# lesliegaga/GPT-SoVITS

Measured on AMD Instinct MI355X. Metric: synthesised audio sec/sec (1/RTF), v2 pipeline, higher is better.
Workload: dtype f16

## Files before the change

### gpt-sovits_amd/csrc/conv_launch.h

```cpp
#pragma once
#include <stdlib.h>

#include <algorithm>
#include <type_traits>

#include "common.h"

namespace gsv {

int launch_gemm_sk(int dtype, const ConvArgs& a, hipStream_t s);
int launch_conv_wide(int dtype, const ConvArgs& a, hipStream_t s);
int launch_gemm_lds(int dtype, const ConvArgs& a, hipStream_t s);
int launch_conv_narrow(int dtype, const ConvArgs& a, hipStream_t s);
int launch_conv_lds(int dtype, const ConvArgs& a, hipStream_t s);

inline const char* env_switch(const char* name) { return getenv(name); }
inline long long env_number(const char* name, long long unset) { const char* v = env_switch(name); return v ? atoll(v) : unset; }
inline char env_first(const char* name) { const char* v = env_switch(name); return v ? v[0] : '\0'; }
struct ConvSwitches {
  bool no_conv_lds = env_switch("GSV_NO_CONV_LDS");
  bool trace_conv_gemm = env_switch("GSV_TRACE_CONV_GEMM");
  long long gemm_small_tiles = env_number("GSV_CONV_GEMM_SMALL_TILES", 64);
  bool no_gemm_sk = env_switch("GSV_NO_GEMM_SK");
  int sk_max_tiles = (int)env_number("GSV_SK_MAX_TILES", 160);
  bool gemm_t64 = env_first("GSV_GEMM_T64") != '0';
  int t64_slab = (int)env_number("GSV_T64_SLAB", 128);
  bool no_conv_wide = env_switch("GSV_NO_CONV_WIDE");
  int wide_waves = (int)env_number("GSV_WIDE_WAVES", 8);
  bool wide_prof = env_switch("GSV_WIDE_PROF");
  int gemm_xcd = env_first("GSV_GEMM_XCD") == '0' ? 0 : env_first("GSV_GEMM_XCD") == '1' ? 1 : 2;
  int gemm_waves = (int)env_number("GSV_GEMM_WAVES", 8);
  long long gemm_w8_max_tiles = env_number("GSV_GEMM_W8_MAX_TILES", 256);
  bool no_persist = env_switch("GSV_CONV_NO_PERSIST");
  bool no_persist64 = env_switch("GSV_CONV_NO_PERSIST64");
  int narrow_per_cu = std::max(1, (int)env_number("GSV_NARROW_PER_CU", 3));
  bool narrow_prof = env_switch("GSV_NARROW_PROF");
  bool no_half_tile = env_switch("GSV_CONV_NO_HALF_TILE");
  bool half_always = env_switch("GSV_CONV_HALF_ALWAYS");
  int half_waves = (int)env_number("GSV_CONV_HALF_WAVES", 8);
  int tile_waves = (int)env_number("GSV_CONV_TILE_WAVES", 8);
  bool no_conv_pair = env_switch("GSV_NO_CONV_PAIR");
  bool no_conv_pair64 = env_switch("GSV_NO_CONV_PAIR64");
  int pair_per_cu = std::max(1, (int)env_number("GSV_PAIR_PER_CU", 3));
};
inline const ConvSwitches& conv_switches() {
  static const ConvSwitches sw{};
  return sw;
}

template <auto Kern, int LdsCap, typename... Args>
int launch_routed(unsigned long long route, dim3 grid, dim3 block, size_t lds, hipStream_t s, Args... args) {
  if constexpr (LdsCap > 0) {
    static bool cap_set = false;
    if (!cap_set) {
      GSV_HIP(hipFuncSetAttribute((const void*)Kern, hipFuncAttributeMaxDynamicSharedMemorySize, LdsCap));
      cap_set = true;
    }
  }
  set_conv_route(route);
  GSV_LAUNCH(Kern, grid, block, lds, s, args...);
  return GSV_OK;
}
constexpr int LDS_CAP = 160 * 1024;

template <typename F> int with_flags(F&& f) { return f(); }
template <typename F, typename... Bools> int with_flags(F&& f, bool b, Bools... rest) {
  return with_flags([&](auto... tail) { return b ? f(std::true_type{}, tail...) : f(std::false_type{}, tail...); }, rest...);
}

template <int G> bool operands_aligned(const ConvArgs& a) {
  return a.ldx % G == 0 && a.ldw % G == 0 && (uintptr_t)a.x % 16 == 0 && (uintptr_t)a.w % 16 == 0;
}

struct TileStamps {
  unsigned long long* dev = nullptr;
  int calls = 0;
  unsigned long long* buffer(bool on) {
    if (on && !dev) { (void)hipMalloc((void**)&dev, 64 * 8); (void)hipMemset(dev, 0, 64 * 8); }
    return dev;
  }
  void report(hipStream_t s, int max_stamps, const char* fmt, ...) {
    if (!dev || ++calls != 3) return;
    (void)hipStreamSynchronize(s);
    unsigned long long hp[64];
    (void)hipMemcpy(hp, dev, sizeof(hp), hipMemcpyDeviceToHost);
    va_list ap;
    va_start(ap, fmt);
    vfprintf(stderr, fmt, ap);
    va_end(ap);
    for (int i = 1; i < max_stamps && hp[i]; ++i) fprintf(stderr, " %.2f", (double)(hp[i] - hp[0]) / 100.0);
    fprintf(stderr, "\n");
  }
};

}
```

### gpt-sovits_amd/csrc/conv_wide.hip

```cpp
#include "conv_launch.h"

namespace gsv {

namespace {

typedef _Float16 T;
typedef h8 F;
typedef _Float16 T4 __attribute__((ext_vector_type(4)));

__device__ __forceinline__ void mma32w(f16v& acc, const h8& a, const h8& b) { acc = __builtin_amdgcn_mfma_f32_32x32x16_f16(a, b, acc, 0, 0, 0); }
__device__ __forceinline__ h8 lrelu8w(h8 v, float s) { h8 t = v * (_Float16)s; return __builtin_elementwise_max(v, t); }
__device__ __forceinline__ h8 relu8w(h8 v) { return __builtin_elementwise_max(v, (h8){0, 0, 0, 0, 0, 0, 0, 0}); }

template <bool RES, bool ACCU, int NW>
__global__ __launch_bounds__(NW * 64) void conv_wide_f16_kernel(ConvArgs a, int rows_win, int ntiles) {
  constexpr int G = 8, KC = 16, CC = 128, CT = 128, TM = 2, TN = NW == 8 ? 2 : 4, WN = NW == 8 ? 4 : 2, NT = NW * 64;
  constexpr int LDX = CC + G, VPR = CC / G;
  constexpr int WLOADS = CT * VPR / NT;
  constexpr int XB = (306 * VPR + NT - 1) / NT;
  constexpr int LDO = CT + 4, PR = TN * 32, IPR = CT / 4, NI = PR * IPR / NT;
  extern __shared__ __attribute__((aligned(16))) unsigned char smem[];
  T* xs = (T*)smem;
  T* ws = xs + (size_t)306 * LDX;
  float* os = (float*)smem;
  static_assert((size_t)PR * LDO * 4 <= (size_t)306 * LDX * 2, "epilogue tile must fit in the window");
  const int tid = threadIdx.x, lane = tid & 63, wave = tid >> 6;
  const int r = lane & 31, h = lane >> 5;
  const int wm = wave / WN, wn = wave % WN;
  const T* __restrict__ x = (const T*)a.x;
  const T* __restrict__ w = (const T*)a.w;
  const int total = rows_win * VPR;
  const int ecg = tid % IPR, ec = 4 * ecg;
  f4 ebias = (f4){0.f, 0.f, 0.f, 0.f};
  if (a.bias) for (int j = 0; j < 4; ++j) ebias[j] = a.bias[ec + j];

  auto load_w = [&](int tap, F* regs) {
#pragma unroll
    for (int i = 0; i < WLOADS; ++i) {
      const int v = tid + i * NT;
      const int row = v / VPR, col = v - row * VPR;
      regs[i] = *(const F*)(w + (long long)row * a.ldw + (long long)tap * CC + col * G);
    }
  };
  auto store_w = [&](int buf, const F* regs) {
#pragma unroll
    for (int i = 0; i < WLOADS; ++i) {
      const int v = tid + i * NT;
      const int row = v / VPR, col = v - row * VPR;
      *(F*)(ws + ((size_t)buf * CT + row) * LDX + col * G) = regs[i];
    }
  };
  auto load_window = [&](int tile, F* regs) {
    const int win_start = tile * 256 - a.pad;
#pragma unroll
    for (int i = 0; i < XB; ++i) {
      const int v = min(tid + i * NT, total - 1);
      const int row = v / VPR, col = v - row * VPR;
      const int ti = win_start + row;
      const F val = *(const F*)(x + (long long)min(max(ti, 0), a.T_in - 1) * a.ldx + col * G);
      regs[i] = (ti >= 0 && ti < a.T_in) ? val : (F){0, 0, 0, 0, 0, 0, 0, 0};
    }
  };
  auto store_window = [&](const F* regs) {
#pragma unroll
    for (int i = 0; i < XB; ++i) {
      const int v = tid + i * NT;
      if (v < total) {
        const int row = v / VPR, col = v - row * VPR;
        F val = regs[i];
        if (a.pre_act == ACT_LRELU) val = lrelu8w(val, a.pre_slope);
        else if (a.pre_act == ACT_RELU) val = relu8w(val);
        *(F*)(xs + (size_t)row * LDX + col * G) = val;
      }
    }
  };
  int tile = blockIdx.x;
  {
    F first[XB], w0[WLOADS];
    load_window(min(tile, ntiles - 1), first);
    load_w(0, w0);
    store_window(first);
    store_w(0, w0);
  }
  lds_barrier();
  for (; tile < ntiles; tile += gridDim.x) {
    const int t0 = tile * 256;
    const bool pf = a.prof && blockIdx.x == 100 && tile == 100 + 3 * (int)gridDim.x && tid == 0;
    int pi = 0;
#define WSTAMP() do { if (pf) a.prof[pi++] = __builtin_amdgcn_s_memrealtime(); } while (0)
    WSTAMP();
    F nxt[XB];
    load_window(min(tile + (int)gridDim.x, ntiles - 1), nxt);
    T4 rv[RES ? NI : 1];
    auto load_res_pass = [&](int pass) {
#pragma unroll
      for (int e = 0; e < (RES ? NI : 0); ++e) {
        const int t = min(t0 + pass * PR + (tid + e * NT) / IPR, a.T_out - 1);
        rv[e] = *(const T4*)((const T*)a.res + (long long)t * a.ldr + ec);
      }
    };
    if (RES) load_res_pass(0);
    f16v acc[TM][TN];
#pragma unroll
    for (int m = 0; m < TM; ++m)
#pragma unroll
      for (int n = 0; n < TN; ++n)
#pragma unroll
        for (int i = 0; i < 16; ++i) acc[m][n][i] = 0.f;
    for (int tap = 0; tap < a.taps; ++tap) {
      const int buf = tap & 1;
      F wnx[WLOADS];
      const bool more = tap + 1 < a.taps;
      if (more) load_w(tap + 1, wnx);
      const int shift = tap * a.dil;
      const T* wb = ws + (size_t)buf * CT * LDX;
#pragma unroll 2
      for (int ks = 0; ks < CC / KC; ++ks) {
        const int kk = ks * KC + G * h;
        F af[TM], bf[TN];
#pragma unroll
        for (int m = 0; m < TM; ++m) af[m] = *(const F*)(wb + (size_t)((wm * TM + m) * 32 + r) * LDX + kk);
#pragma unroll
        for (int n = 0; n < TN; ++n) bf[n] = *(const F*)(xs + (size_t)((wn * TN + n) * 32 + r + shift) * LDX + kk);
#pragma unroll
        for (int m = 0; m < TM; ++m)
#pragma unroll
          for (int n = 0; n < TN; ++n) mma32w(acc[m][n], af[m], bf[n]);
      }
      if (more) {
        store_w(buf ^ 1, wnx);
        lds_barrier();
      }
      WSTAMP();
    }
#pragma unroll
    for (int pass = 0; pass < WN; ++pass) {
      lds_barrier();
      WSTAMP();
      if (wn == pass) {
#pragma unroll
        for (int m = 0; m < TM; ++m)
#pragma unroll
          for (int n = 0; n < TN; ++n) {
            const int tl = n * 32 + r;
#pragma unroll
            for (int g = 0; g < 4; ++g) {
              const int cl = (wm * TM + m) * 32 + 8 * g + 4 * h;
              *(f4*)(os + (size_t)tl * LDO + cl) = (f4){acc[m][n][4 * g], acc[m][n][4 * g + 1], acc[m][n][4 * g + 2], acc[m][n][4 * g + 3]};
            }
          }
      }
      WSTAMP();
      lds_barrier();
      WSTAMP();
      T4 ya[ACCU ? NI : 1];
#pragma unroll
      for (int e = 0; e < (ACCU ? NI : 0); ++e) {
        const int t = min(t0 + pass * PR + (tid + e * NT) / IPR, a.T_out - 1);
        ya[e] = *(const T4*)((const T*)a.y + (long long)t * a.ldy + ec);
      }
      auto items = [&](auto act_tag) {
#pragma unroll
        for (int e = 0; e < NI; ++e) {
          const int tl = (tid + e * NT) / IPR;
          const int t = t0 + pass * PR + tl;
          if (t >= a.T_out) continue;
          const f4 av = *(const f4*)(os + (size_t)tl * LDO + 4 * ecg);
          float v[4];
#pragma unroll
          for (int j = 0; j < 4; ++j) {
            float u = av[j] + ebias[j];
            if (RES) u += (float)rv[e][j];
            u *= a.scale;
            u = post_act_c<decltype(act_tag)::value>(a.post_act, u);
            if (ACCU) u += (float)ya[e][j];
            v[j] = u;
          }
          *(T4*)((T*)a.y + (long long)t * a.ldy + ec) = (T4){(T)v[0], (T)v[1], (T)v[2], (T)v[3]};
        }
      };
      GSV_ACT_DISPATCH(a.post_act, items);
      if (RES && pass + 1 < WN) load_res_pass(pass + 1);
      WSTAMP();
    }
    F w0[WLOADS];
    load_w(0, w0);
    lds_barrier();
    store_window(nxt);
    store_w(0, w0);
    lds_barrier();
    WSTAMP();
  }
}

}

int launch_conv_wide(int dtype, const ConvArgs& a, hipStream_t s) {
  const ConvSwitches& sw = conv_switches();
  if (sw.no_conv_wide || dtype != GSV_F16) return 1;
  if (a.Cin != 128 || a.Cout != 128 || a.Z != 1 || a.stride != 1 || a.ups_u > 0 || a.dil < 1 || a.gate || a.taps < 2) return 1;
  if (a.out_f32 || a.res_f32 || a.y_col0 != 0 || a.T_virt < 16384 || a.T_out != a.T_virt || a.T_in < 1) return 1;
  if (!operands_aligned<8>(a) || a.ldy % 4 != 0 || (a.res && a.ldr % 4 != 0)) return 1;
  const int span = (a.taps - 1) * a.dil;
  if (span > 50 || a.pad < 0 || a.pad > span) return 1;
  const int rows_win = 256 + span;
  const int ntiles = cdiv(a.T_virt, 256);
  const size_t lds = ((size_t)306 + 2 * 128) * 136 * 2;
  const int grid = std::min(ntiles, 256);
  static TileStamps stamps;
  ConvArgs b = a;
  b.prof = stamps.buffer(sw.wide_prof);
  GSV_RC(with_flags([&](auto R, auto A, auto W8) {
    constexpr int NW = W8.value ? 8 : 4;
    return launch_routed<conv_wide_f16_kernel<R.value, A.value, NW>, LDS_CAP>(
        route_code(ROUTE_CONV_WIDE, GSV_F16, NW, 0, 0, 0, 0, route_flags(R.value, A.value)), dim3(grid), dim3(NW * 64), lds, s, b, rows_win, ntiles);
  }, a.res != nullptr, a.accumulate != 0, sw.wide_waves == 8));
  stamps.report(s, 24, "[wide prof] taps %d:", a.taps);
  return GSV_OK;
}

}
```

Before: 2930.

## Give each wave a private epilogue scratch in the wide conv kernel

The block-wide epilogue made 4 passes, each with two block barriers. It is replaced by a per-wave epilogue in which every wave writes its accumulators to its own LDS scratch slice and drains it with only an lgkmcnt wait. Residual and accumulate reads are issued up front for all of a wave's rows. The weight reload for the next tile is folded into the last tap iteration and stored during the epilogue. The 4-wave variant is removed. A non-fused multiply-add is kept for specific elements to preserve exact rounding against a reference, which is an odd numerics-matching hack that adds fragility.

```diff
diff --git a/gpt-sovits_amd/csrc/conv_launch.h b/gpt-sovits_amd/csrc/conv_launch.h
--- a/gpt-sovits_amd/csrc/conv_launch.h
+++ b/gpt-sovits_amd/csrc/conv_launch.h
@@ -26,7 +26,6 @@
   bool gemm_t64 = env_first("GSV_GEMM_T64") != '0';
   int t64_slab = (int)env_number("GSV_T64_SLAB", 128);
   bool no_conv_wide = env_switch("GSV_NO_CONV_WIDE");
-  int wide_waves = (int)env_number("GSV_WIDE_WAVES", 8);
   bool wide_prof = env_switch("GSV_WIDE_PROF");
   int gemm_xcd = env_first("GSV_GEMM_XCD") == '0' ? 0 : env_first("GSV_GEMM_XCD") == '1' ? 1 : 2;
   int gemm_waves = (int)env_number("GSV_GEMM_WAVES", 8);
diff --git a/gpt-sovits_amd/csrc/conv_wide.hip b/gpt-sovits_amd/csrc/conv_wide.hip
--- a/gpt-sovits_amd/csrc/conv_wide.hip
+++ b/gpt-sovits_amd/csrc/conv_wide.hip
@@ -11,33 +11,41 @@
 __device__ __forceinline__ void mma32w(f16v& acc, const h8& a, const h8& b) { acc = __builtin_amdgcn_mfma_f32_32x32x16_f16(a, b, acc, 0, 0, 0); }
 __device__ __forceinline__ h8 lrelu8w(h8 v, float s) { h8 t = v * (_Float16)s; return __builtin_elementwise_max(v, t); }
 __device__ __forceinline__ h8 relu8w(h8 v) { return __builtin_elementwise_max(v, (h8){0, 0, 0, 0, 0, 0, 0, 0}); }
-
-template <bool RES, bool ACCU, int NW>
-__global__ __launch_bounds__(NW * 64) void conv_wide_f16_kernel(ConvArgs a, int rows_win, int ntiles) {
-  constexpr int G = 8, KC = 16, CC = 128, CT = 128, TM = 2, TN = NW == 8 ? 2 : 4, WN = NW == 8 ? 4 : 2, NT = NW * 64;
+__device__ __forceinline__ float mul_then_add(float u, float s, float y) {
+#pragma clang fp contract(off)
+  const float p = u * s;
+  return p + y;
+}
+__device__ __forceinline__ void wave_lds_wait() { asm volatile("s_waitcnt lgkmcnt(0)" ::: "memory"); }
+
+constexpr int WIDE_WAVES = 8;
+template <bool RES, bool ACCU>
+__global__ __launch_bounds__(WIDE_WAVES * 64) void conv_wide_f16_kernel(ConvArgs a, int rows_win, int ntiles) {
+  constexpr int G = 8, KC = 16, CC = 128, CT = 128, TM = 2, TN = 2, WN = 4, NW = WIDE_WAVES, NT = NW * 64;
   constexpr int LDX = CC + G, VPR = CC / G;
   constexpr int WLOADS = CT * VPR / NT;
   constexpr int XB = (306 * VPR + NT - 1) / NT;
-  constexpr int LDO = CT + 4, PR = TN * 32, IPR = CT / 4, NI = PR * IPR / NT;
+  constexpr int WC = TM * 32, HR = 32, LDO = WC + 4, IPR = WC / 4, NI = HR * IPR / 64;
   extern __shared__ __attribute__((aligned(16))) unsigned char smem[];
   T* xs = (T*)smem;
   T* ws = xs + (size_t)306 * LDX;
-  float* os = (float*)smem;
-  static_assert((size_t)PR * LDO * 4 <= (size_t)306 * LDX * 2, "epilogue tile must fit in the window");
+  static_assert((size_t)NW * HR * LDO * 4 <= (size_t)306 * LDX * 2, "the waves' epilogue scratch must fit in the window");
   const int tid = threadIdx.x, lane = tid & 63, wave = tid >> 6;
   const int r = lane & 31, h = lane >> 5;
   const int wm = wave / WN, wn = wave % WN;
+  float* os = (float*)smem + (size_t)wave * HR * LDO;
   const T* __restrict__ x = (const T*)a.x;
   const T* __restrict__ w = (const T*)a.w;
   const int total = rows_win * VPR;
-  const int ecg = tid % IPR, ec = 4 * ecg;
+  const int erow = lane / IPR, ecg = lane % IPR, ec = wm * WC + 4 * ecg;
   f4 ebias = (f4){0.f, 0.f, 0.f, 0.f};
   if (a.bias) for (int j = 0; j < 4; ++j) ebias[j] = a.bias[ec + j];
 
+  int vt = tid;
   auto load_w = [&](int tap, F* regs) {
 #pragma unroll
     for (int i = 0; i < WLOADS; ++i) {
-      const int v = tid + i * NT;
+      const int v = vt + i * NT;
       const int row = v / VPR, col = v - row * VPR;
       regs[i] = *(const F*)(w + (long long)row * a.ldw + (long long)tap * CC + col * G);
     }
@@ -45,7 +53,7 @@
   auto store_w = [&](int buf, const F* regs) {
 #pragma unroll
     for (int i = 0; i < WLOADS; ++i) {
-      const int v = tid + i * NT;
+      const int v = vt + i * NT;
       const int row = v / VPR, col = v - row * VPR;
       *(F*)(ws + ((size_t)buf * CT + row) * LDX + col * G) = regs[i];
     }
@@ -54,7 +62,7 @@
     const int win_start = tile * 256 - a.pad;
 #pragma unroll
     for (int i = 0; i < XB; ++i) {
-      const int v = min(tid + i * NT, total - 1);
+      const int v = min(vt + i * NT, total - 1);
       const int row = v / VPR, col = v - row * VPR;
       const int ti = win_start + row;
       const F val = *(const F*)(x + (long long)min(max(ti, 0), a.T_in - 1) * a.ldx + col * G);
@@ -64,7 +72,7 @@
   auto store_window = [&](const F* regs) {
 #pragma unroll
     for (int i = 0; i < XB; ++i) {
-      const int v = tid + i * NT;
+      const int v = vt + i * NT;
       if (v < total) {
         const int row = v / VPR, col = v - row * VPR;
         F val = regs[i];
@@ -85,21 +93,13 @@
   lds_barrier();
   for (; tile < ntiles; tile += gridDim.x) {
     const int t0 = tile * 256;
+    asm volatile("" : "+v"(vt));
     const bool pf = a.prof && blockIdx.x == 100 && tile == 100 + 3 * (int)gridDim.x && tid == 0;
     int pi = 0;
 #define WSTAMP() do { if (pf) a.prof[pi++] = __builtin_amdgcn_s_memrealtime(); } while (0)
     WSTAMP();
     F nxt[XB];
     load_window(min(tile + (int)gridDim.x, ntiles - 1), nxt);
-    T4 rv[RES ? NI : 1];
-    auto load_res_pass = [&](int pass) {
-#pragma unroll
-      for (int e = 0; e < (RES ? NI : 0); ++e) {
-        const int t = min(t0 + pass * PR + (tid + e * NT) / IPR, a.T_out - 1);
-        rv[e] = *(const T4*)((const T*)a.res + (long long)t * a.ldr + ec);
-      }
-    };
-    if (RES) load_res_pass(0);
     f16v acc[TM][TN];
 #pragma unroll
     for (int m = 0; m < TM; ++m)
@@ -107,11 +107,11 @@
       for (int n = 0; n < TN; ++n)
 #pragma unroll
         for (int i = 0; i < 16; ++i) acc[m][n][i] = 0.f;
+    F wnx[WLOADS];
     for (int tap = 0; tap < a.taps; ++tap) {
       const int buf = tap & 1;
-      F wnx[WLOADS];
       const bool more = tap + 1 < a.taps;
-      if (more) load_w(tap + 1, wnx);
+      load_w(more ? tap + 1 : 0, wnx);
       const int shift = tap * a.dil;
       const T* wb = ws + (size_t)buf * CT * LDX;
 #pragma unroll 2
@@ -133,61 +133,62 @@
       }
       WSTAMP();
     }
-#pragma unroll
-    for (int pass = 0; pass < WN; ++pass) {
-      lds_barrier();
-      WSTAMP();
-      if (wn == pass) {
+    int tw = t0 + wn * (TN * HR) + erow;
+    asm volatile("" : "+v"(tw));
+    T4 rv[RES ? TN * NI : 1], ya[ACCU ? TN * NI : 1];
+#pragma unroll
+    for (int i = 0; i < (RES ? TN * NI : 0); ++i)
+      rv[i] = *(const T4*)((const T*)a.res + (long long)min(tw + 4 * i, a.T_out - 1) * a.ldr + ec);
+    const bool b0_free = (a.taps & 1) == 0;
+    if (b0_free) store_w(0, wnx);
+    lds_barrier();
+    if (!b0_free) store_w(0, wnx);
+#pragma unroll
+    for (int i = 0; i < (ACCU ? TN * NI : 0); ++i)
+      ya[i] = *(const T4*)((const T*)a.y + (long long)min(tw + 4 * i, a.T_out - 1) * a.ldy + ec);
+    WSTAMP();
+    auto epilogue = [&](auto act_tag) {
+      constexpr int ACTC = decltype(act_tag)::value;
+#pragma unroll
+      for (int n = 0; n < TN; ++n) {
 #pragma unroll
         for (int m = 0; m < TM; ++m)
 #pragma unroll
-          for (int n = 0; n < TN; ++n) {
-            const int tl = n * 32 + r;
-#pragma unroll
-            for (int g = 0; g < 4; ++g) {
-              const int cl = (wm * TM + m) * 32 + 8 * g + 4 * h;
-              *(f4*)(os + (size_t)tl * LDO + cl) = (f4){acc[m][n][4 * g], acc[m][n][4 * g + 1], acc[m][n][4 * g + 2], acc[m][n][4 * g + 3]};
-            }
-          }
-      }
-      WSTAMP();
-      lds_barrier();
-      WSTAMP();
-      T4 ya[ACCU ? NI : 1];
-#pragma unroll
-      for (int e = 0; e < (ACCU ? NI : 0); ++e) {
-        const int t = min(t0 + pass * PR + (tid + e * NT) / IPR, a.T_out - 1);
-        ya[e] = *(const T4*)((const T*)a.y + (long long)t * a.ldy + ec);
-      }
-      auto items = [&](auto act_tag) {
+          for (int g = 0; g < 4; ++g)
+            *(f4*)(os + (size_t)r * LDO + m * 32 + 8 * g + 4 * h) = (f4){acc[m][n][4 * g], acc[m][n][4 * g + 1], acc[m][n][4 * g + 2], acc[m][n][4 * g + 3]};
+        wave_lds_wait();
 #pragma unroll
         for (int e = 0; e < NI; ++e) {
-          const int tl = (tid + e * NT) / IPR;
-          const int t = t0 + pass * PR + tl;
+          const int i = n * NI + e;
+          const int t = tw + 4 * i;
           if (t >= a.T_out) continue;
-          const f4 av = *(const f4*)(os + (size_t)tl * LDO + 4 * ecg);
+          const f4 av = *(const f4*)(os + (size_t)(4 * e + erow) * LDO + 4 * ecg);
           float v[4];
 #pragma unroll
           for (int j = 0; j < 4; ++j) {
             float u = av[j] + ebias[j];
-            if (RES) u += (float)rv[e][j];
-            u *= a.scale;
-            u = post_act_c<decltype(act_tag)::value>(a.post_act, u);
-            if (ACCU) u += (float)ya[e][j];
+            if (RES) u += (float)rv[i][j];
+            if (ACCU && ACTC == ACT_NONE) {
+              if (n * HR + 4 * e >= 48 && j == 3) u = mul_then_add(u, a.scale, (float)ya[i][j]);
+              else u = __builtin_fmaf(u, a.scale, (float)ya[i][j]);
+              asm("" : "+v"(u));
+            } else {
+              u *= a.scale;
+              u = post_act_c<ACTC>(a.post_act, u);
+              if (ACCU) u += (float)ya[i][j];
+            }
             v[j] = u;
           }
           *(T4*)((T*)a.y + (long long)t * a.ldy + ec) = (T4){(T)v[0], (T)v[1], (T)v[2], (T)v[3]};
         }
-      };
-      GSV_ACT_DISPATCH(a.post_act, items);
-      if (RES && pass + 1 < WN) load_res_pass(pass + 1);
-      WSTAMP();
-    }
-    F w0[WLOADS];
-    load_w(0, w0);
+        wave_lds_wait();
+        WSTAMP();
+      }
+    };
+    GSV_ACT_DISPATCH(a.post_act, epilogue);
     lds_barrier();
+    WSTAMP();
     store_window(nxt);
-    store_w(0, w0);
     lds_barrier();
     WSTAMP();
   }
@@ -210,11 +211,11 @@
   static TileStamps stamps;
   ConvArgs b = a;
   b.prof = stamps.buffer(sw.wide_prof);
-  GSV_RC(with_flags([&](auto R, auto A, auto W8) {
-    constexpr int NW = W8.value ? 8 : 4;
-    return launch_routed<conv_wide_f16_kernel<R.value, A.value, NW>, LDS_CAP>(
-        route_code(ROUTE_CONV_WIDE, GSV_F16, NW, 0, 0, 0, 0, route_flags(R.value, A.value)), dim3(grid), dim3(NW * 64), lds, s, b, rows_win, ntiles);
-  }, a.res != nullptr, a.accumulate != 0, sw.wide_waves == 8));
+  GSV_RC(with_flags([&](auto R, auto A) {
+    return launch_routed<conv_wide_f16_kernel<R.value, A.value>, LDS_CAP>(
+        route_code(ROUTE_CONV_WIDE, GSV_F16, WIDE_WAVES, 0, 0, 0, 0, route_flags(R.value, A.value)), dim3(grid), dim3(WIDE_WAVES * 64), lds, s, b,
+        rows_win, ntiles);
+  }, a.res != nullptr, a.accumulate != 0));
   stamps.report(s, 24, "[wide prof] taps %d:", a.taps);
   return GSV_OK;
 }
```

Measured after the change: 2957 (median of 6 runs). About the same (+0.9%).
